# jgsimard/big-dreamer

Measured on AMD Instinct MI355X. Metric: latent transitions/sec (RSSM + imagination) at batch=50 chunk=50 H=15, higher is better.
Workload: dtype f32

## Files before the change

big_dreamer_amd/_cabi.py:

```python
from __future__ import annotations

import ctypes as C
import os

import torch

_HERE = os.path.dirname(os.path.abspath(__file__))
LIB_PATH = os.environ.get("BD_LIB") or os.path.join(_HERE, "libbigdreamer_hip.so")

if not os.path.exists(LIB_PATH):
    raise ImportError(
        f"{LIB_PATH} is missing: the MI355X HIP extension has not been built "
        "(run `python -c 'import __graft_entry__ as g; g.build()'`). There is no CPU fallback.")

lib = C.CDLL(LIB_PATH)

BD_MAX_LAYERS = 6
ACT_NONE, ACT_ELU, ACT_ELU_GRAD = 0, 1, 2
P = C.c_void_p
F32 = C.c_float
I32 = C.c_int


class PackDesc(C.Structure):
# ... 182 lines not shown
    "bd_observe_cat_backward": (I32, [C.POINTER(ObserveCatBwdArgs), P]),
    "bd_observe_cat_cluster_size": (I32, [I32, I32, I32, I32, I32]),
    "bd_observe_cat_cluster_ws_floats": (C.c_size_t, [I32, I32, I32, I32, I32]),
    "bd_observe_cat_forward_cluster": (I32, [C.POINTER(ObserveCatFwdArgs), I32, P, C.c_size_t, P]),
    "bd_observe_cat_backward_cluster": (I32, [C.POINTER(ObserveCatBwdArgs), I32, P, C.c_size_t, P]),
    "bd_imagine_cat_forward": (I32, [C.POINTER(ImagineCatFwdArgs), P]),
    "bd_imagine_cat_backward": (I32, [C.POINTER(ImagineCatBwdArgs), P]),
    "bd_imagine_forward": (I32, [C.POINTER(ImagineFwdArgs), P]),
    "bd_imagine_forward_scan": (I32, [C.POINTER(ImagineFwdArgs), P]),
    "bd_actor_entropy": (I32, [P, P, P, I32, I32, I32, I32, P]),
    "bd_imagine_backward": (I32, [C.POINTER(ImagineBwdArgs), P]),
    "bd_lambda_return_forward": (I32, [P, P, I32, I32, F32, F32, P, P]),
    "bd_rng_fill": (I32, [C.POINTER(RngFillArgs), P]),
    "bd_philox4x32_10": (I32, [C.POINTER(C.c_uint), C.POINTER(C.c_uint), C.POINTER(C.c_uint)]),
    "bd_actor_entropy_rng": (I32, [C.c_ulonglong, C.c_ulonglong, C.c_uint, P, P, I32, I32, I32, I32, P]),
    "bd_gemm_nt": (I32, [P, I32, P, I32, P, I32, I32, I32, I32, I32, P]),
    "bd_categorical_head_forward": (I32, [P, P, I32, I32, I32, P, P, P]),
    "bd_categorical_head_backward": (I32, [P, P, I32, I32, I32, P, P]),
    "bd_kl_categorical_forward": (I32, [P, P, I32, I32, I32, F32, I32, P, I32, P, P]),
    "bd_kl_categorical_backward": (I32, [P, P, I32, I32, I32, F32, F32, F32, F32, P, I32, P, P, P]),
    "bd_plan_rollout": (I32, [C.POINTER(PlanArgs), P]),
    "bd_cem_refit": (I32, [P, I32, P, I32, I32, I32, I32, I32, P, P, P]),
    "bd_plan_rollout_cat": (I32, [C.POINTER(PlanCatArgs), P]),
    "bd_lambda_return_backward": (I32, [P, F32, I32, I32, F32, F32, P, P, P]),
    "bd_img_heads_supported": (I32, [I32, I32]),
    "bd_img_heads_fwd_bwd": (I32, [C.POINTER(ImgHeadsArgs), P]),
    "bd_actor_reinforce": (I32, [P, P, P, P, P, P, P, I32, I32, I32, F32, F32, F32, I32, P, P, I32, P, P]),
    "bd_actor_reinforce_cat": (I32, [P, P, P, P, P, P, I32, I32, I32, F32, F32, F32, I32, P, P, I32, P, P]),
    "bd_normal_nll": (I32, [P, I32, P, I32, I32, I32, F32, P, I32, P, I32, P, P]),
    "bd_bernoulli_nll": (I32, [P, P, C.c_size_t, F32, P, P, I32, P, P]),
    "bd_kl_forward": (I32, [P, P, P, P, I32, I32, F32, I32, P, I32, P, P]),
    "bd_kl_backward": (I32, [P, P, P, P, I32, I32, F32, F32, F32, F32, P, I32, P, P, P, P, P]),
    "bd_sum": (I32, [P, C.c_size_t, P, I32, P, P]),
    "bd_sumsq": (I32, [P, C.c_size_t, P, I32, P, P]),
    "bd_adam_step": (I32, [P, P, P, P, C.c_size_t, F32, F32, F32, F32, F32, I32, F32, P, I32, P]),
    "bd_polyak": (I32, [P, P, C.c_size_t, F32, P]),
    "bd_replay_gather": (I32, [P, P, I32, I32, P, P]),
    "bd_replay_gather_pixels": (I32, [P, P, I32, I32, I32, P, P, P]),
    "bd_replay_gather_pixels_rng": (I32, [P, P, I32, I32, I32, C.c_ulonglong, C.c_ulonglong, P, P]),
    "bd_reduce_ws_floats": (C.c_size_t, []),
    "bd_conv_gemm": (I32, [C.POINTER(ConvArgs), P]),
    "bd_conv_thin_forward": (I32, [P, I32, I32, I32, I32, I32, P, I32, P, I32, P, P, P]),
    "bd_conv_pack_class": (I32, [P, P, I32, I32, I32, I32, I32, I32, I32, P]),
    "bd_conv_pack_fused": (I32, [P, P, I32, I32, I32, P]),
    "bd_elu_backward": (I32, [P, P, C.c_size_t, P]),
    "bd_image_layout": (I32, [P, P, I32, I32, I32, I32, P]),
    "bd_colsum_ws_floats": (C.c_size_t, [I32]),
    "bd_colsum": (I32, [P, C.c_size_t, I32, P, P, P]),
}

for _name, (_res, _args) in _SIGS.items():
    _fn = getattr(lib, _name)
    _fn.restype = _res
    _fn.argtypes = _args

# ... 26 lines not shown
```

big_dreamer_amd/csrc/bd_scan.h:

```cpp
#pragma once
#include "bd_device.h"

namespace bd {

struct EntConst {
    float mean, sd, inv_var, inv_sd, base0;
};
__device__ __forceinline__ EntConst entropy_const(float mean, float sd) {
    constexpr float kLogSqrt2Pi = 0.91893853320467274f, kLn2 = 0.69314718055994531f;
    return EntConst{mean, sd, 1.f / (sd * sd), 1.f / sd, -logf(sd) - kLogSqrt2Pi - 2.f * kLn2};
}
__device__ __forceinline__ void entropy_sample(const EntConst& c, float e, float& lp, float& dm, float& ds) {
    constexpr float kClamp = 0.99999994f;
    const float u = c.mean + c.sd * e;
    const float y = tanhf(u);
    const float yc = fminf(fmaxf(y, -kClamp), kClamp);
    const float a = 1.f + yc, b = 1.f - yc;
    const float xh = 0.5f * logf(a / b);
    const float diff = xh - c.mean;
    const float t = -2.f * xh;
    const float ex = expf(t);
    const float sp = t > 20.f ? t : log1pf(ex);
    const float sg = t > 20.f ? 1.f : ex / (1.f + ex);
    lp = c.base0 - 0.5f * diff * diff * c.inv_var + 2.f * (xh + sp);
    const float gx = -diff * c.inv_var + 2.f - 4.f * sg;
    const bool pass = (y >= -kClamp) && (y <= kClamp);
    const float J = pass ? (1.f - y * y) / (a * b) : 0.f;
    dm = diff * c.inv_var + gx * J;
    ds = diff * diff * c.inv_var * c.inv_sd - c.inv_sd + gx * J * e;
}


struct HiddenEpi {
    float* dst;
    float* save;
    size_t tn;
    int width, rows, row0, lane;
    __device__ __forceinline__ void operator()(int nb, floatx4 acc) const {
        const int c = lane & 15, q = lane >> 4;
        float* __restrict__ p = dst + acc_frag_off(nb, lane, 0);
        if (row0 + 16 <= rows && nb * 16 + 16 <= width) {
            float v[4];
#pragma unroll
            for (int r = 0; r < 4; ++r) v[r] = elu(acc[r]);
#pragma unroll
// ... 110 lines not shown
```

big_dreamer_amd/csrc/imagine.hip:

```cpp
#include "bd_device.h"
#include "bd_host.h"
#include "bd_scan.h"
#include "bd_rng.h"
#include "bd_discrete.h"

namespace bd {

constexpr int kMaxA = 64;

#ifdef BD_STAMPS
__device__ unsigned long long g_stamps[64];
#define BD_STAMP(slot)                                                                      \
    do {                                                                                    \
        if (blockIdx.x == BD_STAMP_WG && threadIdx.x == 0 && t == 3) g_stamps[slot] = __builtin_amdgcn_s_memtime(); \
    } while (0)
#ifndef BD_STAMP_WG
#define BD_STAMP_WG 0
#endif
#else
#define BD_STAMP(slot)
#endif

struct ImgDims {
    int Kb_h, Kb_s, Kb_a, Kb_hd;
// ... 236 lines not shown
                        a.prior_std[i] = sd;
                        a.feat[(tn + grow) * F + a.Be + col] = st;
                    }
                    sf[frag_idx(row, col)] = st;
                },
                t == 3 ? 8 : -1);
        }
        BD_STAMP(13);
        lds_barrier();
        BD_STAMP(14);
        float* tmp = h_cur; h_cur = h_nxt; h_nxt = tmp;
    }
#undef a
}

constexpr int kEntParts = 16;
template <bool RNG>
__global__ __launch_bounds__(64 * kEntParts) void actor_entropy_kernel(const float* __restrict__ eps, float* __restrict__ stats,
                                                            float* __restrict__ entropy, int Hm, int N, int A, int ns, Rng rng) {
    __shared__ float red[kEntParts][64][3];
    __shared__ float lpj[64];
    const int lane = threadIdx.x & 63, part = threadIdx.x >> 6;
    const int rows_pb = 64 / A;
    const int rl = lane / A, j = lane - rl * A;
    const long row = (long)blockIdx.x * rows_pb + rl;
    const bool valid = rl < rows_pb && row < (long)Hm * N;
    float lp = 0.f, dm = 0.f, ds = 0.f;
    if (valid) {
        const int t = (int)(row / N), n = (int)(row - (long)t * N);
        const float* st = stats + (size_t)row * 4 * A + j;
        const EntConst ec = entropy_const(st[2 * A], st[3 * A]);
// ... 374 lines not shown
```

big_dreamer_amd/csrc/reduce.hip:

```cpp
#include "bd_device.h"
#include "bd_host.h"
#include "bd_discrete.h"

namespace bd {

constexpr int kRedBlocks = 1024;
constexpr float kHalfLog2Pi = 0.91893853320467274178f;

static inline int red_blocks(size_t n) {
    size_t b = (n + 255) / 256;
    return (int)(b < 1 ? 1 : (b > kRedBlocks ? kRedBlocks : b));
}

__global__ __launch_bounds__(256) void final_sum_kernel(const double* __restrict__ partials, int n,
                                                        float* __restrict__ scalars, int slot) {
    __shared__ double red[kWaves];
    double s = 0.0;
    for (int i = threadIdx.x; i < n; i += blockDim.x) s += partials[i];
    s = block_sum_d(s, red);
    if (threadIdx.x == 0) scalars[slot] = (float)s;
}

template <int MODE>
__global__ __launch_bounds__(256) void sum_kernel(const float* __restrict__ x, size_t n, double* __restrict__ partials) {
// ... 128 lines not shown
                                                             const float* __restrict__ dstate,
                                                             const float* __restrict__ dmean,
                                                             const float* __restrict__ dstd, int M, int S,
                                                             float* __restrict__ dout) {
    const size_t n = (size_t)M * S;
    for (size_t i = (size_t)blockIdx.x * blockDim.x + threadIdx.x; i < n; i += (size_t)gridDim.x * blockDim.x) {
        const size_t r = i / S, c = i - r * S;
        const float ds = dstate ? dstate[i] : 0.f;
        const float gm = ds + (dmean ? dmean[i] : 0.f);
        const float gs = (dstate ? ds * eps[i] : 0.f) + (dstd ? dstd[i] : 0.f);
        dout[r * 2 * S + c] = gm;
        dout[r * 2 * S + S + c] = gs * sigmoidf(out[r * 2 * S + S + c]);
    }
}

__global__ __launch_bounds__(256) void lambda_fwd_kernel(const float* __restrict__ reward, const float* __restrict__ value,
                                                         int Hm, int N, float disc, float lam, float* __restrict__ ret) {
    const float one_minus = 1.f - lam, dl = disc * lam;
    for (int n = blockIdx.x * blockDim.x + threadIdx.x; n < N; n += gridDim.x * blockDim.x) {
        const float boot = value[(size_t)(Hm - 1) * N + n];
        float last = boot;
        for (int t = Hm - 1; t >= 0; --t) {
            const float next = (t == Hm - 1) ? boot : value[(size_t)(t + 1) * N + n];
            const float inp = reward[(size_t)t * N + n] + disc * next * one_minus;
            last = inp + dl * last;
            ret[(size_t)t * N + n] = last;
        }
    }
}

__global__ __launch_bounds__(256) void lambda_bwd_kernel(const float* __restrict__ dret, float dconst, int Hm, int N,
                                                         float disc, float lam, float* __restrict__ dreward,
                                                         float* __restrict__ dvalue) {
    const float c = disc * lam, w = disc * (1.f - lam);
    for (int n = blockIdx.x * blockDim.x + threadIdx.x; n < N; n += gridDim.x * blockDim.x) {
        float G = 0.f;
        for (int t = 0; t < Hm; ++t) {
            G = (dret ? dret[(size_t)t * N + n] : dconst) + c * G;
            dreward[(size_t)t * N + n] = G;
            if (t == 0 && Hm > 1) dvalue[n] = 0.f;
            if (t < Hm - 1) {
                dvalue[(size_t)(t + 1) * N + n] = G * w;
// ... 69 lines not shown
        const float l = __shfl(norm, k, 64);
        float g = c * ((lane == k ? 1.f : 0.f) - p);
        if (write) {
            const float H = disc_entropy(norm, p, valid);
            g += (dentropy * w) * (-p * (norm + H));
        } else if (valid) {
            g += dout[j];
        }
        if (valid) dout[j] = g;
        if (lane == 0) s += (double)(w * l * adv);
    }
    s = block_sum_d(s, red);
    if (threadIdx.x == 0) partials[blockIdx.x] = s;
}

__global__ __launch_bounds__(256) void adam_kernel(float* __restrict__ p, float* __restrict__ g, float* __restrict__ m,
                                                   float* __restrict__ v, size_t n, float beta1, float beta2, float eps,
                                                   float wd, float step_size, float inv_sqrt_bc2, float max_norm,
                                                   const float* __restrict__ scalars, int sqnorm_slot) {
    const float total_norm = sqrtf(scalars[sqnorm_slot]);
    const float q = max_norm / (total_norm + 1e-6f);
    const float coef = q > 1.f ? 1.f : q;
    for (size_t i = (size_t)blockIdx.x * blockDim.x + threadIdx.x; i < n; i += (size_t)gridDim.x * blockDim.x) {
        const float gc = g[i] * coef;
        g[i] = gc;
        const float pi = p[i];
        const float gw = gc + wd * pi;
        const float mi = m[i] + (1.f - beta1) * (gw - m[i]);
        const float vi = v[i] * beta2 + (1.f - beta2) * gw * gw;
        m[i] = mi;
        v[i] = vi;
        const float denom = sqrtf(vi) * inv_sqrt_bc2 + eps;
        p[i] = pi - step_size * (mi / denom);
    }
}

__global__ __launch_bounds__(256) void polyak_kernel(float* __restrict__ t, const float* __restrict__ s, size_t n, float w) {
    for (size_t i = (size_t)blockIdx.x * blockDim.x + threadIdx.x; i < n; i += (size_t)gridDim.x * blockDim.x)
        t[i] = s[i] * w + t[i] * (1.f - w);
}

constexpr int kCatPer = 4;

__device__ __forceinline__ float half_max(float v) {
#pragma unroll
    for (int o = 16; o > 0; o >>= 1) v = fmaxf(v, __shfl_xor(v, o, 64));
    return v;
}
__device__ __forceinline__ float half_sum(float v) {
// ... 159 lines not shown
            group_log_softmax(pl + base, C, l, lp);
            const float kl = group_kl(lq, lp, C, l);
#pragma unroll
            for (int i = 0; i < kCatPer; ++i) {
                const int c = l + 32 * i;
                if (c < C) {
                    const float qv = expf(lq[i]), pv = expf(lp[i]);
                    dql[base + c] = f * fq * (qv == 0.f ? 0.f : qv * (lq[i] - lp[i] - kl));
                    dpl[base + c] = f * fp * (pv - qv);
                }
            }
        }
    }
}

static int finish(double* partials, int nb, float* scalars, int slot, hipStream_t s, const char* name) {
    hipLaunchKernelGGL(final_sum_kernel, dim3(1), dim3(256), 0, s, partials, nb, scalars, slot);
    BD_CHECK_LAUNCH(name);
    return 0;
}

}

extern "C" {
using namespace bd;

size_t bd_reduce_ws_floats(void) { return 2 * (size_t)kRedBlocks; }

int bd_sum(const float* x, size_t n, float* scalars, int slot, float* ws, void* stream) {
    BD_REQUIRE(x && scalars && ws && n > 0, "bd_sum: bad arguments");
    const int nb = red_blocks(n);
    hipLaunchKernelGGL(sum_kernel<0>, dim3(nb), dim3(256), 0, (hipStream_t)stream, x, n, (double*)ws);
    BD_CHECK_LAUNCH("bd_sum");
    return finish((double*)ws, nb, scalars, slot, (hipStream_t)stream, "bd_sum(final)");
}

int bd_actor_reinforce(const float* eps_action, const float* act_us, const float* act_stats, const float* returns,
                       const float* base0, const float* value, const float* weight, int Hm, int N, int A, float rho,
                       float grad_scale, float dentropy, int write, float* d_actor_out, float* scalars, int slot, float* ws,
                       void* stream) {
    BD_REQUIRE(eps_action && act_us && act_stats && returns && base0 && (value || Hm == 1) && d_actor_out && scalars && ws,
               "bd_actor_reinforce: missing pointers");
// ... 91 lines not shown
    hipLaunchKernelGGL(gauss_head_bwd_kernel, dim3(red_blocks((size_t)M * S)), dim3(256), 0, (hipStream_t)stream, out, eps,
                       dstate, dmean, dstd, M, S, dout);
    BD_CHECK_LAUNCH("bd_gauss_head_backward");
    return 0;
}

int bd_lambda_return_forward(const float* reward, const float* value, int Hm, int N, float discount, float lambda_,
                             float* returns, void* stream) {
    BD_REQUIRE(reward && value && returns && Hm > 0 && N > 0, "bd_lambda_return_forward: bad arguments");
    hipLaunchKernelGGL(lambda_fwd_kernel, dim3(red_blocks(N)), dim3(256), 0, (hipStream_t)stream, reward, value, Hm, N,
                       discount, lambda_, returns);
    BD_CHECK_LAUNCH("bd_lambda_return_forward");
    return 0;
}

int bd_lambda_return_backward(const float* dreturns, float dret_const, int Hm, int N, float discount, float lambda_,
                              float* dreward, float* dvalue, void* stream) {
    BD_REQUIRE(dreward && dvalue && Hm > 0 && N > 0, "bd_lambda_return_backward: bad arguments");
    hipLaunchKernelGGL(lambda_bwd_kernel, dim3(red_blocks(N)), dim3(256), 0, (hipStream_t)stream, dreturns, dret_const, Hm,
                       N, discount, lambda_, dreward, dvalue);
    BD_CHECK_LAUNCH("bd_lambda_return_backward");
    return 0;
}

int bd_adam_step(float* p, float* g, float* m, float* v, size_t n, float lr, float beta1, float beta2, float eps,
                 float weight_decay, int step, float max_norm, const float* scalars, int sqnorm_slot, void* stream) {
    BD_REQUIRE(p && g && m && v && scalars && n > 0 && step >= 1, "bd_adam_step: bad arguments");
    const double bc1 = 1.0 - pow((double)beta1, step), bc2 = 1.0 - pow((double)beta2, step);
    hipLaunchKernelGGL(adam_kernel, dim3(red_blocks(n)), dim3(256), 0, (hipStream_t)stream, p, g, m, v, n, beta1, beta2,
                       eps, weight_decay, (float)(lr / bc1), (float)(1.0 / sqrt(bc2)), max_norm, scalars, sqnorm_slot);
    BD_CHECK_LAUNCH("bd_adam_step");
    return 0;
}

int bd_polyak(float* target, const float* src, size_t n, float weight, void* stream) {
    BD_REQUIRE(target && src && n > 0, "bd_polyak: bad arguments");
    hipLaunchKernelGGL(polyak_kernel, dim3(red_blocks(n)), dim3(256), 0, (hipStream_t)stream, target, src, n, weight);
    BD_CHECK_LAUNCH("bd_polyak");
    return 0;
}

static inline int cat_blocks(size_t units) {
    size_t b = (units + 7) / 8;
    return (int)(b < 1 ? 1 : (b > (size_t)kRedBlocks ? (size_t)kRedBlocks : b));
}

// ... 49 lines not shown
```

big_dreamer_amd/engine.py:

```python
from __future__ import annotations

import collections.abc
import ctypes as C
import math
import os
import weakref
from typing import Dict, List, Optional, Tuple

import numpy as np
import torch

from . import _cabi as cabi
from .parallel import DataParallel
from .params import ParamGroup, _adam_state_dict, _load_adam_state_dict
from .synth import DENSE_LAYERS, MODEL_MODULES, Dims, model_modules, param_shapes

lib = cabi.lib
ptr = cabi.ptr

DEFAULT_HP = dict(
    kl_balance=0.8, kl_loss_weight=0.1, free_nats=3.0, grad_clip_norm=100.0, discount=0.995, disclam=0.95,
    model_learning_rate=2e-4, actor_learning_rate=4e-5, value_learning_rate=1e-4, adam_epsilon=1e-5,
    weight_decay=1e-6, entropy_weight=1e-5, polyak_avg=1.0, min_std_dev=0.1, discount_weight=5.0,
    gradient_mixing=-1,
# ... 158 lines not shown
            torch.cuda.synchronize(self.dev)
        d = dims
        shapes = param_shapes(d)
        self.groups = {
            "model": ParamGroup([(m, n, s) for m in model_modules(d) for n, s in shapes[m]], self.dev,
                                conv_storage=self.pixel),
            "actor": ParamGroup([("actor", n, s) for n, s in shapes["actor"]], self.dev),
            "critic": ParamGroup([("critic", n, s) for n, s in shapes["critic"]], self.dev),
            "critic_target": ParamGroup([("critic_target", n, s) for n, s in shapes["critic"]], self.dev, False),
        }
        self._mod_group = {m: "model" for m in model_modules(d)}
        self._mod_group.update(actor="actor", critic="critic", critic_target="critic_target")
        if params is not None:
            self.load_params(params)
        self.scalars = torch.zeros(N_SLOTS, dtype=torch.float32, device=self.dev)
        self.red_ws = torch.zeros(int(lib.bd_reduce_ws_floats()), dtype=torch.float32, device=self.dev)
        self._wgrad_ws = torch.zeros(1, dtype=torch.float32, device=self.dev)
        self._wgrad_ws_side = torch.zeros(1, dtype=torch.float32, device=self.dev)
        self._wgrad_ws_early = torch.zeros(1, dtype=torch.float32, device=self.dev)
        self.red_ws_side = torch.zeros(int(lib.bd_reduce_ws_floats()), dtype=torch.float32, device=self.dev)
        self._wbatch = {"model": WgradBatch(self, "model"), "model_early": WgradBatch(self, "model_early", "_wgrad_ws_early"),
                        "actor": WgradBatch(self, "actor", "_wgrad_ws_bh"),
                        "critic": WgradBatch(self, "critic", "_wgrad_ws_side")}
        self._side = _engine_stream(self.dev, "side", int(os.environ.get("BD_SIDE_PRIO", "0")))
        self.heads_fused = (os.environ.get("BD_HEADS_FUSED", "1") != "0" and not self.d.categorical
                            and bool(lib.bd_img_heads_supported(self.d.Be + self.d.S, self.d.Hd)))
        self._s_early = _engine_stream(self.dev, "early", int(os.environ.get("BD_EARLY_PRIO", "0")))
        self.pipeline = os.environ.get("BD_PIPELINE", "1") != "0"
        self._s_wm = _engine_stream(self.dev, "wm", int(os.environ.get("BD_WM_PRIO", "-1")))
        bh_prio = int(os.environ.get("BD_BH_PRIO", "0" if self.pixel else "-1"))
        self._s_bh = _engine_stream(self.dev, "bh", bh_prio)
# ... 7 lines not shown
            self.defer_opt = shared_comm or os.environ.get("BD_DEFER_OPT", "0") == "1"
        if (world_size > 1 or self.dp.force) and torch.cuda.current_stream(self.dev) == torch.cuda.default_stream(self.dev):
            self._main_stream = _engine_stream(self.dev, "main", 0)
            torch.cuda.set_stream(self._main_stream)
        self._pending_opt: List[tuple] = []
        self._opt_over: Dict[str, dict] = {}
        self._rng_seed: Optional[int] = None
        self._rng_step = {"wm": 0, "bh": 0}
        self._rng_entropy_step = 0
        self._log_ring: List[_LogRecord] = []
        self._log_i = 0
        self._cur_rec: Optional[_LogRecord] = None
        self._wm_done_hist: List[torch.cuda.Event] = []
        self._parity = 0
        self._wgrad_ws_bh = torch.zeros(1, dtype=torch.float32, device=self.dev)
        self.red_ws_bh = torch.zeros(int(lib.bd_reduce_ws_floats()), dtype=torch.float32, device=self.dev)
        self._buf: Dict[str, torch.Tensor] = {}
        self.host_ahead = int(os.environ.get("BD_HOST_AHEAD", "2"))
        self._bh_hist: List["torch.cuda.Event"] = []
        self.use_obs_cluster = os.environ.get("BD_OBS_CLUSTER", "1") != "0"
        self._obs_ws: Optional[torch.Tensor] = None
        self._obs_err_off: Optional[int] = None
        self._timers_on, self._timer_every, self._timer_tick = False, 1, 0
        self._timer_events: Dict[str, List[Tuple[torch.cuda.Event, torch.cuda.Event]]] = {}
        self._build_pack_tables()
        self.conv = None
        if self.pixel:
            from .conv_stack import ConvStacks
            self.conv = ConvStacks(self)
        for g in ("model", "actor", "critic", "critic_target"):
            self.pack(g)

# ... 219 lines not shown

    def _allreduce(self, t: torch.Tensor, key: Optional[str] = None) -> None:
        self.dp.allreduce_sum_(t, key)

    def optimizer_step(self, group: str, slot: int, lr: float, red_ws: Optional[torch.Tensor] = None,
                       rec: Optional[_LogRecord] = None) -> None:
        g = self.groups[group]
        red_ws = self.red_ws if red_ws is None else red_ws
        self._allreduce(g.grad, group)
        g.step += 1
        hp = self.hp
        ov = self._opt_over.get(group)
        if ov:
            lr = ov.get("lr", lr)
        eps, wd = (ov or {}).get("eps", hp["adam_epsilon"]), (ov or {}).get("weight_decay", hp["weight_decay"])
        cabi.check(lib.bd_sumsq(ptr(g.grad), g.numel, ptr(self.scalars), slot, ptr(red_ws), cabi.stream()))
        cabi.check(lib.bd_adam_step(ptr(g.flat), ptr(g.grad), ptr(g.m), ptr(g.v), g.numel, lr, 0.9, 0.999,
                                    eps, wd, g.step, hp["grad_clip_norm"],
                                    ptr(self.scalars), slot, cabi.stream()))
        self.pack(group)
        rec = rec if rec is not None else self._cur_rec
        if rec is not None:
            self._snapshot(rec, _LogRecord.ROW[group])

    def _new_record(self) -> _LogRecord:
        if len(self._log_ring) < 8:
            self._log_ring.append(_LogRecord())
            rec = self._log_ring[-1]
        else:
            rec = self._log_ring[self._log_i]
            self._log_i = (self._log_i + 1) % 8
            owner = rec.owner() if rec.owner is not None else None
            if owner is not None and owner._vals is None:
                owner.resolve()
# ... 267 lines not shown
        pk = self.pk
        a.w_a0h = ptr(pk["a0h"])
        for l in range(1, DENSE_LAYERS):
            a.w_a[l - 1] = ptr(pk[f"a{l}"])
        for l in range(DENSE_LAYERS):
            a.b_a[l] = ptr(self.W("actor", f"model.{2 * l}.bias"))
        a.b_a4 = ptr(self.W("actor", f"model.{2 * DENSE_LAYERS}.bias"))
        if self.d.discrete_actions:
            a.w_a4m, a.w_a4s, a.discrete_actions = ptr(pk["a4"]), None, 1
        else:
            a.w_a4m, a.w_a4s = ptr(pk["a4m"]), ptr(pk["a4s"])

    def _entropy_estimate(self, noise, ent: torch.Tensor, Hm: int, N: int) -> None:
        d = self.d
        if noise.get("entropy") is not None:
            cabi.check(lib.bd_actor_entropy(ptr(noise["entropy"]), ptr(self._buf["sv_act_stats"]), ptr(ent), Hm, N, d.A,
                                            d.n_entropy, cabi.stream()))
        else:
            cabi.check(lib.bd_actor_entropy_rng(self.rng_seed, self._rng_entropy_step, self.RNG_STREAMS["entropy"],
                                                ptr(self._buf["sv_act_stats"]), ptr(ent), Hm, N, d.A, d.n_entropy, cabi.stream()))

    def plan(self, belief: torch.Tensor, state: torch.Tensor, horizon: int, iters: int, candidates: int, top: int,
             eps_action: torch.Tensor, eps_state: Optional[torch.Tensor], trace: Optional[list] = None) -> torch.Tensor:
        d, pk = self.d, self.pk
        tm = lambda n: self.W("transition_model", n)
        B = belief.shape[0]
        rows = B * candidates
        cat = d.categorical
        mean = self.buf("plan_mean", horizon, B, d.A)
        std = self.buf("plan_std", horizon, B, d.A)
        mean.zero_()
        std.fill_(1.0)
        actions = self.buf("plan_actions", horizon, rows, d.A)
        returns = self.buf("plan_returns", rows)
# ... 422 lines not shown
            arr[:, 0] = 1.0
            wts = self.buf(ptag + "disc_w", Mi)
            wts.view(Hm, N).copy_(torch.cumprod(arr, 0))
            if mix is None:
                dret = self.buf("dret_w", Mi)
                torch.mul(wts, -inv_mi, out=dret)
            elif dyn:
                dret = self.buf("dret_w", Mi)
                torch.mul(wts, -mix * inv_mi, out=dret)
        fused = dyn and self.heads_fused
        if dyn:
            d_r, d_v = self.buf("d_ir_out", Mi), self.buf("d_iv_out", Mi)
            dconst = -inv_mi if mix is None else -mix * inv_mi
            difeat = self.buf("difeat", Mi, F)
        if fused:
            cabi.check(lib.bd_lambda_return_backward(ptr(dret), dconst, Hm, N, hp["discount"], hp["disclam"], ptr(d_r),
                                                     ptr(d_v), st))
            r_out, v_out = self.buf("ir_out", Mi, 1), self.buf("iv_out", Mi, 1)
            with self.span("img_heads_bwd"):
                self.img_heads_fused(Mi, ifeat, d_r, d_v, r_out, v_out, difeat)
        else:
            with self.span("img_heads_fwd"):
                r_out, r_acts, r_layers = self.dense_forward("reward_model", "rew", "ir", ifeat, F, Mi, 1, sidx=isidx)
                v_out, v_acts, v_layers = self.dense_forward("critic_target", "tgt", "iv", ifeat, F, Mi, 1, sidx=isidx)
        returns = self.buf(ptag + "returns", Mi)
        cabi.check(lib.bd_lambda_return_forward(ptr(r_out), ptr(v_out), Hm, N, hp["discount"], hp["disclam"], ptr(returns), st))
        cabi.check(lib.bd_sum(ptr(returns), Mi, sc, SLOT_RET, ws, st))
        cabi.check(lib.bd_sum(ptr(ent), Mi, sc, SLOT_ENT, ws, st))
        if d.use_discount:
            ew_ = hp["entropy_weight"] if hp["entropy_weight"] != -1 else 0.0
            if mix is None:
                self.scalars[SLOT_WOBJ] = (wts * (returns + ew_ * ent)).sum()
            else:
                self.scalars[SLOT_WOBJ] = (wts * (mix * returns + ew_ * ent)).sum()
        if par is not None:
            ev_ret = torch.cuda.Event()
            ev_ret.record(torch.cuda.current_stream())
            with torch.cuda.stream(self._side):
                self._side.wait_event(ev_ret)
                self._critic_phase(ifeat, returns, Mi, F, inv_mi, self.red_ws_side, isidx, wts)
                self._ev_cr_done[par] = torch.cuda.Event()
                self._ev_cr_done[par].record(self._side)
        dentropy = -hp["entropy_weight"] * inv_mi if hp["entropy_weight"] != -1 else 0.0
        d_apre, d_aout = self.buf("d_actor_pre", DENSE_LAYERS, Mi, d.Hd), self.buf("d_actor_out", Mi, d.actor_out)
        sv_actor = self._buf["sv_actor"]
        actor_chain = os.environ.get("BD_ACTOR_BWD_CHAIN", "1") == "1" or mix is not None or d.discrete_actions
        if dyn:
            if not fused:
                cabi.check(lib.bd_lambda_return_backward(ptr(dret), dconst, Hm, N, hp["discount"], hp["disclam"],
                                                         ptr(d_r), ptr(d_v), st))
                with self.span("img_heads_bwd"):
                    self.mlp_backward(Mi, d_r, 1, r_layers, r_acts + [None], None, din0=difeat, ld0=F, w0=F)
                    self.mlp_backward(Mi, d_v, 1, v_layers, v_acts + [None], None, din0=difeat, ld0=F, w0=F,
                                      accumulate=True)
            if d.categorical:
                c = cabi.ImagineCatBwdArgs()
                c.N, c.Hm, c.Be, c.D, c.C, c.A, c.Hd = N, Hm, d.Be, d.cat_D, d.cat_C, d.A, d.Hd
                c.wt_p2 = ptr(pk["p2.T"])
                c.prior_logits = ptr(self._buf["iprior_logits"])
            else:
                c = cabi.ImagineBwdArgs()
                c.N, c.Hm, c.Be, c.S, c.A, c.Hd = N, Hm, d.Be, d.S, d.A, d.Hd
                c.wt_p2m, c.wt_p2s = ptr(pk["p2m.T"]), ptr(pk["p2s.T"])
                c.prior_std, c.eps_prior, c.min_std = ptr(self._buf["iprior_std"]), ptr(noise["img_prior"]), hp["min_std_dev"]
            self._bind_rssm_t(c)
# ... 39 lines not shown
        wa = self._wbatch["actor"]
        wa.add(d_apre[0], d.Hd, feat, F, Mi, d.Hd, F, Ga("model.0.weight"), F, Ga("model.0.bias"), act2=ifeat, lda2=F, M1=N)
        for l in range(1, DENSE_LAYERS):
            wa.add(d_apre[l], d.Hd, sv_actor[l - 1], d.Hd, Mi, d.Hd, d.Hd, Ga(f"model.{2 * l}.weight"), d.Hd,
                   Ga(f"model.{2 * l}.bias"))
        wa.add(d_aout, d.actor_out, sv_actor[DENSE_LAYERS - 1], d.Hd, Mi, d.actor_out, d.Hd,
               Ga(f"model.{2 * DENSE_LAYERS}.weight"), d.Hd, Ga(f"model.{2 * DENSE_LAYERS}.bias"))
        with self.span("wgrad_actor"):
            wa.run()
        self._optimizer_step_or_defer("opt_actor", "actor", SLOT_GN_ACTOR, hp["actor_learning_rate"], red_ws)

        if par is None:
            self._critic_phase(ifeat, returns, Mi, F, inv_mi, red_ws, isidx, wts)
        self._counts = dict(N=N, Mi=Mi, S=(d.cat_D if d.categorical else d.S), sum_form=sum_form)

    def _critic_phase(self, ifeat, returns, Mi: int, F: int, inv_mi: float, red_ws: torch.Tensor, isidx=None, wts=None) -> None:
        d, hp = self.d, self.hp
        st, sc = cabi.stream(), ptr(self.scalars)
        with self.span("critic_fwd_bwd"):
            c_out, c_acts, c_layers = self.dense_forward("critic", "cri", "ic", ifeat, F, Mi, 1, sidx=isidx)
            d_c = self.buf("d_ic_out", Mi, 1)
            cabi.check(lib.bd_normal_nll(ptr(c_out), 1, ptr(returns), 1, Mi, 1, inv_mi, ptr(d_c), 1, sc, SLOT_VAL, ptr(red_ws), st))
            if wts is not None:
                d_c.view(Mi).mul_(wts)
                diff = c_out.view(Mi) - returns
                self.scalars[SLOT_VAL] = (wts * (0.5 * diff * diff + 0.9189385332046727)).sum()
            c_dpre = [self.buf(f"ic_dpre{l}", Mi, d.Hd) for l in range(DENSE_LAYERS)] + [d_c]
            self.mlp_backward(Mi, d_c, 1, c_layers, c_acts + [None], c_dpre[:-1] + [None])
        wc = self._wbatch["critic"]
        self._dense_wgrads(wc, "critic", Mi, c_dpre, ifeat, F, c_acts, [F] + [d.Hd] * DENSE_LAYERS + [1])
# ... 55 lines not shown
```

include/bigdreamer_hip.h:

```cpp
#ifndef BIGDREAMER_HIP_H
#define BIGDREAMER_HIP_H

#include <stddef.h>
#include <stdint.h>

#ifdef __cplusplus
extern "C" {
#endif

#define BD_MAX_LAYERS 6
#define BD_ACT_NONE 0
#define BD_ACT_ELU 1
#define BD_ACT_ELU_GRAD 2

const char* bd_last_error(void);
int bd_version(void);

typedef struct {
    const float* src;
    float* dst;
    int ld;
    int N, K;
    int transpose;
} bd_pack_desc;
// ... 193 lines not shown
    const float* eps_action; const float* eps_prior;
    const float* sv_actor; const float* sv_act_stats; const float* sv_x; const float* sv_gates;
    const float* sv_p;
    float min_std;
    const float* dfeat;
    float dentropy;
    float* d_actor_pre;
    float* d_actor_out;
    const float* ent_weight;
    int discrete_actions;
} bd_imagine_bwd_args;
int bd_imagine_backward(const bd_imagine_bwd_args* a, void* stream);

int bd_lambda_return_forward(const float* reward, const float* value, int Hm, int N, float discount,
                             float lambda_, float* returns, void* stream);
int bd_lambda_return_backward(const float* dreturns, float dret_const, int Hm, int N, float discount,
                              float lambda_, float* dreward, float* dvalue, void* stream);

#define BD_HEAD_HIDDEN 4
typedef struct {
    const float* w[BD_HEAD_HIDDEN];
    const float* wt[BD_HEAD_HIDDEN];
    const float* b[BD_HEAD_HIDDEN];
    const float* w_out;
    const float* b_out;
    const float* dout;
    float* out;
} bd_img_head;
typedef struct {
    int M, F, Hd;
// ... 19 lines not shown
typedef struct {
    int n;
    unsigned long long seed;
    unsigned long long step;
    struct {
        float* p;
        size_t count;
        int kind;
        unsigned stream_id;
    } t[BD_RNG_MAX_TENSORS];
} bd_rng_fill_args;
int bd_rng_fill(const bd_rng_fill_args* a, void* stream);
int bd_philox4x32_10(const unsigned* ctr4, const unsigned* key2, unsigned* out4);
int bd_actor_entropy_rng(unsigned long long seed, unsigned long long step, unsigned stream_id, float* act_stats,
                         float* entropy, int Hm, int N, int A, int n_samples, void* stream);

int bd_gemm_nt(const float* A, int lda, const float* B, int ldb, float* C, int ldc, int M, int N, int K, int accumulate,
               void* stream);

int bd_categorical_head_forward(const float* logits, const float* q_noise, int rows, int D, int C, float* state,
                                float* probs, void* stream);
int bd_categorical_head_backward(const float* dstate, const float* probs, int rows, int D, int C, float* dlogits,
                                 void* stream);
int bd_kl_categorical_forward(const float* post_logits, const float* prior_logits, int rows, int D, int C, float free_nats,
                              int sum_form, float* scalars, int slot, float* ws, void* stream);
int bd_kl_categorical_backward(const float* post_logits, const float* prior_logits, int rows, int D, int C, float free_nats,
                               float kl_balance, float weight, float inv_count, const float* scalars, int slot,
                               float* dpost, float* dprior, void* stream);

typedef struct {
// ... 142 lines not shown
                  float grad_scale, float* dpred, int ldd, float* scalars, int slot, float* ws, void* stream);
int bd_bernoulli_nll(const float* logits, const float* target, size_t n, float grad_scale, float* dlogits, float* scalars,
                     int slot, float* ws, void* stream);

int bd_kl_forward(const float* qm, const float* qs, const float* pm, const float* ps, int rows, int S,
                  float free_nats, int sum_form, float* scalars, int slot, float* ws, void* stream);
int bd_kl_backward(const float* qm, const float* qs, const float* pm, const float* ps, int rows, int S,
                   float free_nats, float kl_balance, float weight, float inv_count, const float* scalars,
                   int slot, float* dqm, float* dqs, float* dpm, float* dps, void* stream);
int bd_sum(const float* x, size_t n, float* scalars, int slot, float* ws, void* stream);
int bd_sumsq(const float* x, size_t n, float* scalars, int slot, float* ws, void* stream);

int bd_adam_step(float* p, float* g, float* m, float* v, size_t n, float lr, float beta1, float beta2,
                 float eps, float weight_decay, int step, float max_norm, const float* scalars,
                 int sqnorm_slot, void* stream);
int bd_polyak(float* target, const float* src, size_t n, float weight, void* stream);

int bd_replay_gather(const float* src, const int64_t* idx, int n_idx, int width, float* dst, void* stream);

int bd_replay_gather_pixels(const unsigned char* src, const int64_t* idx, int n_idx, int pixels, int bit_depth,
                            const float* noise, float* dst, void* stream);
int bd_replay_gather_pixels_rng(const unsigned char* src, const int64_t* idx, int n_idx, int pixels, int bit_depth,
                                unsigned long long seed, unsigned long long step, float* dst, void* stream);

size_t bd_reduce_ws_floats(void);

#ifdef __cplusplus
}
#endif
#endif
```

Baseline: 13.11 million.

## Fuse clip into Adam, lambda-return with sums, group entropy kernel, skip redundant dret

Several independent changes. The gradient-norm final reduction is folded into the Adam update kernel, so each block re-reduces the partials instead of running a separate final-sum launch. The lambda-return forward is fused with the return and entropy sums when discounting is off. A 256-thread grouped entropy kernel, with 16 lanes per row, replaces the 1024-thread one. The constant-gradient lambda-return backward is skipped when its arguments match the previous call. Costs are redundant per-block partial reductions and a cache key that depends on buffer pointers.

```diff
diff --git a/big_dreamer_amd/_cabi.py b/big_dreamer_amd/_cabi.py
--- a/big_dreamer_amd/_cabi.py
+++ b/big_dreamer_amd/_cabi.py
@@ -220,6 +220,8 @@
     "bd_rng_fill": (I32, [C.POINTER(RngFillArgs), P]),
     "bd_philox4x32_10": (I32, [C.POINTER(C.c_uint), C.POINTER(C.c_uint), C.POINTER(C.c_uint)]),
     "bd_actor_entropy_rng": (I32, [C.c_ulonglong, C.c_ulonglong, C.c_uint, P, P, I32, I32, I32, I32, P]),
+    "bd_actor_entropy_grouped": (I32, [P, P, P, I32, I32, I32, I32, P]),
+    "bd_actor_entropy_rng_grouped": (I32, [C.c_ulonglong, C.c_ulonglong, C.c_uint, P, P, I32, I32, I32, I32, P]),
     "bd_gemm_nt": (I32, [P, I32, P, I32, P, I32, I32, I32, I32, I32, P]),
     "bd_categorical_head_forward": (I32, [P, P, I32, I32, I32, P, P, P]),
     "bd_categorical_head_backward": (I32, [P, P, I32, I32, I32, P, P]),
@@ -228,6 +230,7 @@
     "bd_plan_rollout": (I32, [C.POINTER(PlanArgs), P]),
     "bd_cem_refit": (I32, [P, I32, P, I32, I32, I32, I32, I32, P, P, P]),
     "bd_plan_rollout_cat": (I32, [C.POINTER(PlanCatArgs), P]),
+    "bd_lambda_return_forward_sums": (I32, [P, P, P, I32, I32, F32, F32, P, P, I32, I32, P, P]),
     "bd_lambda_return_backward": (I32, [P, F32, I32, I32, F32, F32, P, P, P]),
     "bd_img_heads_supported": (I32, [I32, I32]),
     "bd_img_heads_fwd_bwd": (I32, [C.POINTER(ImgHeadsArgs), P]),
@@ -240,11 +243,13 @@
     "bd_sum": (I32, [P, C.c_size_t, P, I32, P, P]),
     "bd_sumsq": (I32, [P, C.c_size_t, P, I32, P, P]),
     "bd_adam_step": (I32, [P, P, P, P, C.c_size_t, F32, F32, F32, F32, F32, I32, F32, P, I32, P]),
+    "bd_clip_adam_step": (I32, [P, P, P, P, C.c_size_t, F32, F32, F32, F32, F32, I32, F32, P, I32, P, P]),
     "bd_polyak": (I32, [P, P, C.c_size_t, F32, P]),
     "bd_replay_gather": (I32, [P, P, I32, I32, P, P]),
     "bd_replay_gather_pixels": (I32, [P, P, I32, I32, I32, P, P, P]),
     "bd_replay_gather_pixels_rng": (I32, [P, P, I32, I32, I32, C.c_ulonglong, C.c_ulonglong, P, P]),
     "bd_reduce_ws_floats": (C.c_size_t, []),
+    "bd_reduce_ws_pair_floats": (C.c_size_t, []),
     "bd_conv_gemm": (I32, [C.POINTER(ConvArgs), P]),
     "bd_conv_thin_forward": (I32, [P, I32, I32, I32, I32, I32, P, I32, P, I32, P, P, P]),
     "bd_conv_pack_class": (I32, [P, P, I32, I32, I32, I32, I32, I32, I32, P]),
diff --git a/big_dreamer_amd/csrc/bd_scan.h b/big_dreamer_amd/csrc/bd_scan.h
--- a/big_dreamer_amd/csrc/bd_scan.h
+++ b/big_dreamer_amd/csrc/bd_scan.h
@@ -29,6 +29,8 @@
     dm = diff * c.inv_var + gx * J;
     ds = diff * diff * c.inv_var * c.inv_sd - c.inv_sd + gx * J * e;
 }
+
+constexpr int kEntParts = 16;
 
 
 struct HiddenEpi {
diff --git a/big_dreamer_amd/csrc/imagine.hip b/big_dreamer_amd/csrc/imagine.hip
--- a/big_dreamer_amd/csrc/imagine.hip
+++ b/big_dreamer_amd/csrc/imagine.hip
@@ -274,7 +274,6 @@
 #undef a
 }
 
-constexpr int kEntParts = 16;
 template <bool RNG>
 __global__ __launch_bounds__(64 * kEntParts) void actor_entropy_kernel(const float* __restrict__ eps, float* __restrict__ stats,
                                                             float* __restrict__ entropy, int Hm, int N, int A, int ns, Rng rng) {
diff --git a/big_dreamer_amd/csrc/reduce.hip b/big_dreamer_amd/csrc/reduce.hip
--- a/big_dreamer_amd/csrc/reduce.hip
+++ b/big_dreamer_amd/csrc/reduce.hip
@@ -1,6 +1,8 @@
 #include "bd_device.h"
 #include "bd_host.h"
 #include "bd_discrete.h"
+#include "bd_rng.h"
+#include "bd_scan.h"
 
 namespace bd {
 
@@ -166,6 +168,17 @@
     }
 }
 
+__device__ __forceinline__ float lambda_step(float reward, float next, float last, float disc, float one_minus, float dl,
+                                             bool first) {
+#pragma clang fp contract(off)
+    const float x = disc * next;
+    if (first) {
+        const float inp = reward + x * one_minus;
+        return inp + dl * last;
+    }
+    return __builtin_fmaf(dl, last, __builtin_fmaf(x, one_minus, reward));
+}
+
 __global__ __launch_bounds__(256) void lambda_fwd_kernel(const float* __restrict__ reward, const float* __restrict__ value,
                                                          int Hm, int N, float disc, float lam, float* __restrict__ ret) {
     const float one_minus = 1.f - lam, dl = disc * lam;
@@ -174,10 +187,47 @@
         float last = boot;
         for (int t = Hm - 1; t >= 0; --t) {
             const float next = (t == Hm - 1) ? boot : value[(size_t)(t + 1) * N + n];
-            const float inp = reward[(size_t)t * N + n] + disc * next * one_minus;
-            last = inp + dl * last;
+            last = lambda_step(reward[(size_t)t * N + n], next, last, disc, one_minus, dl, t == Hm - 1);
             ret[(size_t)t * N + n] = last;
         }
+    }
+}
+
+__global__ __launch_bounds__(256) void lambda_fwd_sums_kernel(const float* __restrict__ reward,
+                                                              const float* __restrict__ value,
+                                                              const float* __restrict__ entropy, int Hm, int N, float disc,
+                                                              float lam, float* __restrict__ ret,
+                                                              double* __restrict__ partials) {
+    __shared__ double red[kWaves];
+    const float one_minus = 1.f - lam, dl = disc * lam;
+    double sr = 0.0, se = 0.0;
+    for (int n = blockIdx.x * blockDim.x + threadIdx.x; n < N; n += gridDim.x * blockDim.x) {
+        const float boot = value[(size_t)(Hm - 1) * N + n];
+        float last = boot;
+        for (int t = Hm - 1; t >= 0; --t) {
+            const float next = (t == Hm - 1) ? boot : value[(size_t)(t + 1) * N + n];
+            last = lambda_step(reward[(size_t)t * N + n], next, last, disc, one_minus, dl, t == Hm - 1);
+            ret[(size_t)t * N + n] = last;
+            sr += (double)last;
+            se += (double)entropy[(size_t)t * N + n];
+        }
+    }
+    sr = block_sum_d(sr, red);
+    se = block_sum_d(se, red);
+    if (threadIdx.x == 0) {
+        partials[blockIdx.x] = sr;
+        partials[kRedBlocks + blockIdx.x] = se;
+    }
+}
+
+__global__ __launch_bounds__(256) void two_sums_kernel(const double* __restrict__ partials, int n,
+                                                       float* __restrict__ scalars, int slot0, int slot1) {
+    __shared__ double red[kWaves];
+    for (int h = 0; h < 2; ++h) {
+        double s = 0.0;
+        for (int i = threadIdx.x; i < n; i += blockDim.x) s += partials[h * kRedBlocks + i];
+        s = block_sum_d(s, red);
+        if (threadIdx.x == 0) scalars[h ? slot1 : slot0] = (float)s;
     }
 }
 
@@ -277,11 +327,10 @@
     if (threadIdx.x == 0) partials[blockIdx.x] = s;
 }
 
-__global__ __launch_bounds__(256) void adam_kernel(float* __restrict__ p, float* __restrict__ g, float* __restrict__ m,
-                                                   float* __restrict__ v, size_t n, float beta1, float beta2, float eps,
-                                                   float wd, float step_size, float inv_sqrt_bc2, float max_norm,
-                                                   const float* __restrict__ scalars, int sqnorm_slot) {
-    const float total_norm = sqrtf(scalars[sqnorm_slot]);
+__device__ __forceinline__ void adam_update(float* __restrict__ p, float* __restrict__ g, float* __restrict__ m,
+                                            float* __restrict__ v, size_t n, float beta1, float beta2, float eps, float wd,
+                                            float step_size, float inv_sqrt_bc2, float max_norm, float sqnorm) {
+    const float total_norm = sqrtf(sqnorm);
     const float q = max_norm / (total_norm + 1e-6f);
     const float coef = q > 1.f ? 1.f : q;
     for (size_t i = (size_t)blockIdx.x * blockDim.x + threadIdx.x; i < n; i += (size_t)gridDim.x * blockDim.x) {
@@ -296,6 +345,31 @@
         const float denom = sqrtf(vi) * inv_sqrt_bc2 + eps;
         p[i] = pi - step_size * (mi / denom);
     }
+}
+
+__global__ __launch_bounds__(256) void adam_kernel(float* __restrict__ p, float* __restrict__ g, float* __restrict__ m,
+                                                   float* __restrict__ v, size_t n, float beta1, float beta2, float eps,
+                                                   float wd, float step_size, float inv_sqrt_bc2, float max_norm,
+                                                   const float* __restrict__ scalars, int sqnorm_slot) {
+    adam_update(p, g, m, v, n, beta1, beta2, eps, wd, step_size, inv_sqrt_bc2, max_norm, scalars[sqnorm_slot]);
+}
+
+__global__ __launch_bounds__(256) void clip_adam_kernel(float* __restrict__ p, float* __restrict__ g, float* __restrict__ m,
+                                                        float* __restrict__ v, size_t n, float beta1, float beta2, float eps,
+                                                        float wd, float step_size, float inv_sqrt_bc2, float max_norm,
+                                                        const double* __restrict__ partials, int np,
+                                                        float* __restrict__ scalars, int sqnorm_slot) {
+    __shared__ double red[kWaves];
+    __shared__ float sqnorm;
+    double s = 0.0;
+    for (int i = threadIdx.x; i < np; i += blockDim.x) s += partials[i];
+    s = block_sum_d(s, red);
+    if (threadIdx.x == 0) {
+        sqnorm = (float)s;
+        if (blockIdx.x == 0) scalars[sqnorm_slot] = (float)s;
+    }
+    __syncthreads();
+    adam_update(p, g, m, v, n, beta1, beta2, eps, wd, step_size, inv_sqrt_bc2, max_norm, sqnorm);
 }
 
 __global__ __launch_bounds__(256) void polyak_kernel(float* __restrict__ t, const float* __restrict__ s, size_t n, float w) {
@@ -485,6 +559,61 @@
     }
 }
 
+template <bool RNG>
+__global__ __launch_bounds__(256) void actor_entropy_group_kernel(const float* __restrict__ eps, float* __restrict__ stats,
+                                                                  float* __restrict__ entropy, int Hm, int N, int A, int ns,
+                                                                  Rng rng) {
+    static_assert(kEntParts == 16, "one group = 16 adjacent lanes");
+    const int part = threadIdx.x & (kEntParts - 1);
+    const long row = (long)blockIdx.x * (256 / kEntParts) + (threadIdx.x >> 4);
+    const bool valid = row < (long)Hm * N;
+    const int t = valid ? (int)(row / N) : 0, n = valid ? (int)(row - (long)t * N) : 0;
+    const float inv_ns = 1.f / (float)ns;
+    float ent = 0.f;
+    for (int j = 0; j < A; ++j) {
+        float lp = 0.f, dm = 0.f, ds = 0.f;
+        if (valid) {
+            const float* st = stats + (size_t)row * 4 * A + j;
+            const EntConst ec = entropy_const(st[2 * A], st[3 * A]);
+            if constexpr (RNG) {
+                const int mine = (ns - part + kEntParts - 1) / kEntParts;
+                const uint64_t base = (((uint64_t)row * A + j) * kEntParts + part) * (uint64_t)((ns / kEntParts + 4) / 4);
+                for (int k0 = 0; k0 < mine; k0 += 4) {
+                    float e[4];
+                    rng_normal4(rng, base + (k0 >> 2), e);
+#pragma unroll
+                    for (int q = 0; q < 4; ++q)
+                        if (k0 + q < mine) {
+                            float l1, d1, d2;
+                            entropy_sample(ec, e[q], l1, d1, d2);
+                            lp += l1; dm += d1; ds += d2;
+                        }
+                }
+            } else {
+                const float* e0 = eps + ((size_t)t * ns * N + n) * A + j;
+                for (int k = part; k < ns; k += kEntParts) {
+                    float l1, d1, d2;
+                    entropy_sample(ec, e0[(size_t)k * N * A], l1, d1, d2);
+                    lp += l1; dm += d1; ds += d2;
+                }
+            }
+        }
+#pragma unroll
+        for (int o = kEntParts / 2; o > 0; o >>= 1) {
+            lp += __shfl_xor(lp, o, 64);
+            dm += __shfl_xor(dm, o, 64);
+            ds += __shfl_xor(ds, o, 64);
+        }
+        if (valid && part == 0) {
+            float* st = stats + (size_t)row * 4 * A + j;
+            st[2 * A] = -dm * inv_ns;
+            st[3 * A] = -ds * inv_ns;
+        }
+        ent += lp;
+    }
+    if (valid && part == 0) entropy[row] = -ent * inv_ns;
+}
+
 static int finish(double* partials, int nb, float* scalars, int slot, hipStream_t s, const char* name) {
     hipLaunchKernelGGL(final_sum_kernel, dim3(1), dim3(256), 0, s, partials, nb, scalars, slot);
     BD_CHECK_LAUNCH(name);
@@ -497,6 +626,7 @@
 using namespace bd;
 
 size_t bd_reduce_ws_floats(void) { return 2 * (size_t)kRedBlocks; }
+size_t bd_reduce_ws_pair_floats(void) { return 4 * (size_t)kRedBlocks; }
 
 int bd_sum(const float* x, size_t n, float* scalars, int slot, float* ws, void* stream) {
     BD_REQUIRE(x && scalars && ws && n > 0, "bd_sum: bad arguments");
@@ -618,6 +748,21 @@
     return 0;
 }
 
+int bd_lambda_return_forward_sums(const float* reward, const float* value, const float* entropy, int Hm, int N,
+                                  float discount, float lambda_, float* returns, float* scalars, int slot_ret, int slot_ent,
+                                  float* ws, void* stream) {
+    BD_REQUIRE(reward && value && entropy && returns && scalars && ws && Hm > 0 && N > 0 && slot_ret >= 0 && slot_ent >= 0,
+               "bd_lambda_return_forward_sums: bad arguments");
+    const int nb = red_blocks(N);
+    hipLaunchKernelGGL(lambda_fwd_sums_kernel, dim3(nb), dim3(256), 0, (hipStream_t)stream, reward, value, entropy, Hm, N,
+                       discount, lambda_, returns, (double*)ws);
+    BD_CHECK_LAUNCH("bd_lambda_return_forward_sums");
+    hipLaunchKernelGGL(two_sums_kernel, dim3(1), dim3(256), 0, (hipStream_t)stream, (const double*)ws, nb, scalars, slot_ret,
+                       slot_ent);
+    BD_CHECK_LAUNCH("bd_lambda_return_forward_sums(final)");
+    return 0;
+}
+
 int bd_lambda_return_backward(const float* dreturns, float dret_const, int Hm, int N, float discount, float lambda_,
                               float* dreward, float* dvalue, void* stream) {
     BD_REQUIRE(dreward && dvalue && Hm > 0 && N > 0, "bd_lambda_return_backward: bad arguments");
@@ -634,6 +779,45 @@
     hipLaunchKernelGGL(adam_kernel, dim3(red_blocks(n)), dim3(256), 0, (hipStream_t)stream, p, g, m, v, n, beta1, beta2,
                        eps, weight_decay, (float)(lr / bc1), (float)(1.0 / sqrt(bc2)), max_norm, scalars, sqnorm_slot);
     BD_CHECK_LAUNCH("bd_adam_step");
+    return 0;
+}
+
+int bd_clip_adam_step(float* p, float* g, float* m, float* v, size_t n, float lr, float beta1, float beta2, float eps,
+                      float weight_decay, int step, float max_norm, float* scalars, int sqnorm_slot, float* ws,
+                      void* stream) {
+    BD_REQUIRE(p && g && m && v && scalars && ws && n > 0 && step >= 1 && sqnorm_slot >= 0, "bd_clip_adam_step: bad arguments");
+    const int nb = red_blocks(n);
+    hipLaunchKernelGGL(sum_kernel<1>, dim3(nb), dim3(256), 0, (hipStream_t)stream, g, n, (double*)ws);
+    BD_CHECK_LAUNCH("bd_clip_adam_step(sumsq)");
+    const double bc1 = 1.0 - pow((double)beta1, step), bc2 = 1.0 - pow((double)beta2, step);
+    hipLaunchKernelGGL(clip_adam_kernel, dim3(nb), dim3(256), 0, (hipStream_t)stream, p, g, m, v, n, beta1, beta2, eps,
+                       weight_decay, (float)(lr / bc1), (float)(1.0 / sqrt(bc2)), max_norm, (const double*)ws, nb, scalars,
+                       sqnorm_slot);
+    BD_CHECK_LAUNCH("bd_clip_adam_step");
+    return 0;
+}
+
+int bd_actor_entropy_grouped(const float* eps_entropy, float* act_stats, float* entropy, int Hm, int N, int A, int n_samples,
+                             void* stream) {
+    BD_REQUIRE(eps_entropy && act_stats && entropy && Hm > 0 && N > 0 && A > 0 && n_samples > 0 &&
+                   (size_t)Hm * N <= (size_t)INT32_MAX / 4,
+               "bd_actor_entropy_grouped: bad arguments");
+    const int rows = Hm * N;
+    hipLaunchKernelGGL(actor_entropy_group_kernel<false>, dim3((rows + 15) / 16), dim3(256), 0, (hipStream_t)stream,
+                       eps_entropy, act_stats, entropy, Hm, N, A, n_samples, Rng{0, 0, 0, 0});
+    BD_CHECK_LAUNCH("bd_actor_entropy_grouped");
+    return 0;
+}
+
+int bd_actor_entropy_rng_grouped(unsigned long long seed, unsigned long long step, unsigned stream_id, float* act_stats,
+                                 float* entropy, int Hm, int N, int A, int n_samples, void* stream) {
+    BD_REQUIRE(act_stats && entropy && Hm > 0 && N > 0 && A > 0 && n_samples > 0 && (size_t)Hm * N <= (size_t)INT32_MAX / 4,
+               "bd_actor_entropy_rng_grouped: bad arguments");
+    const int rows = Hm * N;
+    hipLaunchKernelGGL(actor_entropy_group_kernel<true>, dim3((rows + 15) / 16), dim3(256), 0, (hipStream_t)stream, nullptr,
+                       act_stats, entropy, Hm, N, A, n_samples,
+                       Rng{(uint32_t)seed, (uint32_t)(seed >> 32), stream_id, (uint32_t)step});
+    BD_CHECK_LAUNCH("bd_actor_entropy_rng_grouped");
     return 0;
 }
 
diff --git a/big_dreamer_amd/engine.py b/big_dreamer_amd/engine.py
--- a/big_dreamer_amd/engine.py
+++ b/big_dreamer_amd/engine.py
@@ -196,7 +196,7 @@
         if params is not None:
             self.load_params(params)
         self.scalars = torch.zeros(N_SLOTS, dtype=torch.float32, device=self.dev)
-        self.red_ws = torch.zeros(int(lib.bd_reduce_ws_floats()), dtype=torch.float32, device=self.dev)
+        self.red_ws = torch.zeros(int(lib.bd_reduce_ws_pair_floats()), dtype=torch.float32, device=self.dev)
         self._wgrad_ws = torch.zeros(1, dtype=torch.float32, device=self.dev)
         self._wgrad_ws_side = torch.zeros(1, dtype=torch.float32, device=self.dev)
         self._wgrad_ws_early = torch.zeros(1, dtype=torch.float32, device=self.dev)
@@ -234,8 +234,9 @@
         self._wm_done_hist: List[torch.cuda.Event] = []
         self._parity = 0
         self._wgrad_ws_bh = torch.zeros(1, dtype=torch.float32, device=self.dev)
-        self.red_ws_bh = torch.zeros(int(lib.bd_reduce_ws_floats()), dtype=torch.float32, device=self.dev)
+        self.red_ws_bh = torch.zeros(int(lib.bd_reduce_ws_pair_floats()), dtype=torch.float32, device=self.dev)
         self._buf: Dict[str, torch.Tensor] = {}
+        self._dret_key = None
         self.host_ahead = int(os.environ.get("BD_HOST_AHEAD", "2"))
         self._bh_hist: List["torch.cuda.Event"] = []
         self.use_obs_cluster = os.environ.get("BD_OBS_CLUSTER", "1") != "0"
@@ -485,10 +486,9 @@
         if ov:
             lr = ov.get("lr", lr)
         eps, wd = (ov or {}).get("eps", hp["adam_epsilon"]), (ov or {}).get("weight_decay", hp["weight_decay"])
-        cabi.check(lib.bd_sumsq(ptr(g.grad), g.numel, ptr(self.scalars), slot, ptr(red_ws), cabi.stream()))
-        cabi.check(lib.bd_adam_step(ptr(g.flat), ptr(g.grad), ptr(g.m), ptr(g.v), g.numel, lr, 0.9, 0.999,
-                                    eps, wd, g.step, hp["grad_clip_norm"],
-                                    ptr(self.scalars), slot, cabi.stream()))
+        cabi.check(lib.bd_clip_adam_step(ptr(g.flat), ptr(g.grad), ptr(g.m), ptr(g.v), g.numel, lr, 0.9, 0.999,
+                                         eps, wd, g.step, hp["grad_clip_norm"],
+                                         ptr(self.scalars), slot, ptr(red_ws), cabi.stream()))
         self.pack(group)
         rec = rec if rec is not None else self._cur_rec
         if rec is not None:
@@ -786,10 +786,10 @@
     def _entropy_estimate(self, noise, ent: torch.Tensor, Hm: int, N: int) -> None:
         d = self.d
         if noise.get("entropy") is not None:
-            cabi.check(lib.bd_actor_entropy(ptr(noise["entropy"]), ptr(self._buf["sv_act_stats"]), ptr(ent), Hm, N, d.A,
+            cabi.check(lib.bd_actor_entropy_grouped(ptr(noise["entropy"]), ptr(self._buf["sv_act_stats"]), ptr(ent), Hm, N, d.A,
                                             d.n_entropy, cabi.stream()))
         else:
-            cabi.check(lib.bd_actor_entropy_rng(self.rng_seed, self._rng_entropy_step, self.RNG_STREAMS["entropy"],
+            cabi.check(lib.bd_actor_entropy_rng_grouped(self.rng_seed, self._rng_entropy_step, self.RNG_STREAMS["entropy"],
                                                 ptr(self._buf["sv_act_stats"]), ptr(ent), Hm, N, d.A, d.n_entropy, cabi.stream()))
 
     def plan(self, belief: torch.Tensor, state: torch.Tensor, horizon: int, iters: int, candidates: int, top: int,
@@ -1242,8 +1242,7 @@
             dconst = -inv_mi if mix is None else -mix * inv_mi
             difeat = self.buf("difeat", Mi, F)
         if fused:
-            cabi.check(lib.bd_lambda_return_backward(ptr(dret), dconst, Hm, N, hp["discount"], hp["disclam"], ptr(d_r),
-                                                     ptr(d_v), st))
+            self._lambda_return_backward(dret, dconst, Hm, N, d_r, d_v)
             r_out, v_out = self.buf("ir_out", Mi, 1), self.buf("iv_out", Mi, 1)
             with self.span("img_heads_bwd"):
                 self.img_heads_fused(Mi, ifeat, d_r, d_v, r_out, v_out, difeat)
@@ -1252,9 +1251,13 @@
                 r_out, r_acts, r_layers = self.dense_forward("reward_model", "rew", "ir", ifeat, F, Mi, 1, sidx=isidx)
                 v_out, v_acts, v_layers = self.dense_forward("critic_target", "tgt", "iv", ifeat, F, Mi, 1, sidx=isidx)
         returns = self.buf(ptag + "returns", Mi)
-        cabi.check(lib.bd_lambda_return_forward(ptr(r_out), ptr(v_out), Hm, N, hp["discount"], hp["disclam"], ptr(returns), st))
-        cabi.check(lib.bd_sum(ptr(returns), Mi, sc, SLOT_RET, ws, st))
-        cabi.check(lib.bd_sum(ptr(ent), Mi, sc, SLOT_ENT, ws, st))
+        if d.use_discount:
+            cabi.check(lib.bd_lambda_return_forward(ptr(r_out), ptr(v_out), Hm, N, hp["discount"], hp["disclam"], ptr(returns), st))
+            cabi.check(lib.bd_sum(ptr(returns), Mi, sc, SLOT_RET, ws, st))
+            cabi.check(lib.bd_sum(ptr(ent), Mi, sc, SLOT_ENT, ws, st))
+        else:
+            cabi.check(lib.bd_lambda_return_forward_sums(ptr(r_out), ptr(v_out), ptr(ent), Hm, N, hp["discount"],
+                                                         hp["disclam"], ptr(returns), sc, SLOT_RET, SLOT_ENT, ws, st))
         if d.use_discount:
             ew_ = hp["entropy_weight"] if hp["entropy_weight"] != -1 else 0.0
             if mix is None:
@@ -1275,8 +1278,7 @@
         actor_chain = os.environ.get("BD_ACTOR_BWD_CHAIN", "1") == "1" or mix is not None or d.discrete_actions
         if dyn:
             if not fused:
-                cabi.check(lib.bd_lambda_return_backward(ptr(dret), dconst, Hm, N, hp["discount"], hp["disclam"],
-                                                         ptr(d_r), ptr(d_v), st))
+                self._lambda_return_backward(dret, dconst, Hm, N, d_r, d_v)
                 with self.span("img_heads_bwd"):
                     self.mlp_backward(Mi, d_r, 1, r_layers, r_acts + [None], None, din0=difeat, ld0=F, w0=F)
                     self.mlp_backward(Mi, d_v, 1, v_layers, v_acts + [None], None, din0=difeat, ld0=F, w0=F,
@@ -1346,6 +1348,16 @@
             self._critic_phase(ifeat, returns, Mi, F, inv_mi, red_ws, isidx, wts)
         self._counts = dict(N=N, Mi=Mi, S=(d.cat_D if d.categorical else d.S), sum_form=sum_form)
 
+    def _lambda_return_backward(self, dret: Optional[torch.Tensor], dconst: float, Hm: int, N: int, d_r: torch.Tensor,
+                                d_v: torch.Tensor) -> None:
+        hp = self.hp
+        key = None if dret is not None else (Hm, N, hp["discount"], hp["disclam"], dconst, d_r.data_ptr(), d_v.data_ptr())
+        if key is not None and key == self._dret_key:
+            return
+        cabi.check(lib.bd_lambda_return_backward(ptr(dret), dconst, Hm, N, hp["discount"], hp["disclam"], ptr(d_r),
+                                                 ptr(d_v), cabi.stream()))
+        self._dret_key = key
+
     def _critic_phase(self, ifeat, returns, Mi: int, F: int, inv_mi: float, red_ws: torch.Tensor, isidx=None, wts=None) -> None:
         d, hp = self.d, self.hp
         st, sc = cabi.stream(), ptr(self.scalars)
diff --git a/include/bigdreamer_hip.h b/include/bigdreamer_hip.h
--- a/include/bigdreamer_hip.h
+++ b/include/bigdreamer_hip.h
@@ -231,6 +231,9 @@
 
 int bd_lambda_return_forward(const float* reward, const float* value, int Hm, int N, float discount,
                              float lambda_, float* returns, void* stream);
+int bd_lambda_return_forward_sums(const float* reward, const float* value, const float* entropy, int Hm, int N,
+                                  float discount, float lambda_, float* returns, float* scalars, int slot_ret,
+                                  int slot_ent, float* ws, void* stream);
 int bd_lambda_return_backward(const float* dreturns, float dret_const, int Hm, int N, float discount,
                               float lambda_, float* dreward, float* dvalue, void* stream);
 
@@ -280,6 +283,10 @@
 int bd_philox4x32_10(const unsigned* ctr4, const unsigned* key2, unsigned* out4);
 int bd_actor_entropy_rng(unsigned long long seed, unsigned long long step, unsigned stream_id, float* act_stats,
                          float* entropy, int Hm, int N, int A, int n_samples, void* stream);
+int bd_actor_entropy_grouped(const float* eps_entropy, float* act_stats, float* entropy, int Hm, int N, int A,
+                             int n_samples, void* stream);
+int bd_actor_entropy_rng_grouped(unsigned long long seed, unsigned long long step, unsigned stream_id, float* act_stats,
+                                 float* entropy, int Hm, int N, int A, int n_samples, void* stream);
 
 int bd_gemm_nt(const float* A, int lda, const float* B, int ldb, float* C, int ldc, int M, int N, int K, int accumulate,
                void* stream);
@@ -452,6 +459,9 @@
 int bd_adam_step(float* p, float* g, float* m, float* v, size_t n, float lr, float beta1, float beta2,
                  float eps, float weight_decay, int step, float max_norm, const float* scalars,
                  int sqnorm_slot, void* stream);
+int bd_clip_adam_step(float* p, float* g, float* m, float* v, size_t n, float lr, float beta1, float beta2, float eps,
+                      float weight_decay, int step, float max_norm, float* scalars, int sqnorm_slot, float* ws,
+                      void* stream);
 int bd_polyak(float* target, const float* src, size_t n, float weight, void* stream);
 
 int bd_replay_gather(const float* src, const int64_t* idx, int n_idx, int width, float* dst, void* stream);
@@ -462,6 +472,7 @@
                                 unsigned long long seed, unsigned long long step, float* dst, void* stream);
 
 size_t bd_reduce_ws_floats(void);
+size_t bd_reduce_ws_pair_floats(void);
 
 #ifdef __cplusplus
 }
```

After: 13.26 million (median of 2 runs). No clear change (+1.2%).
